# sashajenner/honours

Hardware: AMD Instinct MI355X
Metric: raw-signal MB/s (compress+decompress) (higher is better)
Workload: dtype u16

## Files before the change

honours_amd/csrc/press_huffman.hip:

```cpp

#include "press_internal.h"
#include "press_packed.h"
#include "press_wave.h"
#include <cstddef>
#include <type_traits>

namespace ph {

#ifdef HUF_STAMPS
__device__ unsigned long long g_hstamp[32];
#define HSTAMP_DECL                                             \
	unsigned long long hs_t = __builtin_amdgcn_s_memtime(); \
	unsigned long long hs_acc[8] = { 0, 0, 0, 0, 0, 0, 0, 0 }
#define HSTAMP(i)                                                              \
	do {     \
		__builtin_amdgcn_sched_barrier(0);                             \
		const unsigned long long hs_n = __builtin_amdgcn_s_memtime(); \
		hs_acc[(i) & 7] += hs_n - hs_t;                                \
		hs_t = hs_n;                                                   \
		__builtin_amdgcn_sched_barrier(0);                             \
	} while (0)
#define HSTAMP_FLUSH(base)                                                     \
	do {                                                                   \
		if ((threadIdx.x & 63) == 0)                                   \
			for (int hs_i = 0; hs_i < 8; hs_i++)                   \
				atomicAdd(&g_hstamp[(base) + hs_i], hs_acc[hs_i]); \
	} while (0)
#else
#define HSTAMP_DECL
#define HSTAMP(i)
#define HSTAMP_FLUSH(base)
#endif

constexpr uint32_t HEND = 0xFFFFFFFFu;
constexpr uint32_t R_END = 31;
constexpr int HT = HUF_HT;

__device__ __forceinline__ uint32_t uniform(uint32_t v) { return (uint32_t) __builtin_amdgcn_readfirstlane((int) v); }
__device__ __forceinline__ bool any64(bool c) { return __builtin_amdgcn_ballot_w64(c) != 0; }

__device__ __noinline__ uint32_t trie_code(const HuffDev *hd, uint32_t wnd)
{
	int node = 0;
	uint32_t l = 0;
	while (node >= 0 && hd->leaf[node] < 0 && l < 32) {
		node = hd->child[node][(wnd >> l) & 1u];
		l++;
	}
	if (node < 0 || hd->leaf[node] < 0)
		return 0;
	return (uint32_t) hd->leaf[node] | (l << 8) | (l << 24);
}

template <int RU>
struct HufGeo {
	static constexpr int OWN = 2 * RU;
	static constexpr int NDW = OWN / 32 + 1;
	static constexpr int NCOL = NDW + 1;
};

__device__ __forceinline__ uint32_t clamp_nb(int64_t v)
{
	return v <= 0 ? 0u : (v > 0x7FFFFFFF ? 0x7FFFFFFFu : (uint32_t) v);
}

#ifndef HUF_NO_NT
__device__ __forceinline__ uint4 ld16_pay(const uint8_t *p)
{
	typedef uint32_t u32x4_u __attribute__((ext_vector_type(4), aligned(1)));
	const u32x4_u v = __builtin_nontemporal_load(reinterpret_cast<const u32x4_u *>(p));
	return make_uint4(v.x, v.y, v.z, v.w);
}
__device__ __forceinline__ uint32_t ld4_pay(const uint8_t *p)
{
	typedef uint32_t __attribute__((aligned(1))) u32_u;
	return __builtin_nontemporal_load(reinterpret_cast<const u32_u *>(p));
}
#else
__device__ __forceinline__ uint4 ld16_pay(const uint8_t *p)
{
	uint4 v;
	__builtin_memcpy(&v, p, 16);
	return v;
}
__device__ __forceinline__ uint32_t ld4_pay(const uint8_t *p)
{
	uint32_t v;
	__builtin_memcpy(&v, p, 4);
	return v;
}
#endif

template <int NDW, int S = 64>
__device__ __forceinline__ void col_load(uint32_t *col, const uint8_t *src, int32_t rb0, int32_t lo, int32_t nby)
{
	if (rb0 >= lo && rb0 + 4 * NDW <= nby) {
		const uint8_t *q = src + rb0;
		uint4 t[NDW / 4 ? NDW / 4 : 1];
		uint32_t x[NDW % 4 ? NDW % 4 : 1];
#pragma unroll
		for (int j = 0; j < NDW / 4; j++)
			t[j] = ld16_pay(q + 16 * j);
#pragma unroll
		for (int j = 0; j < NDW % 4; j++)
			x[j] = ld4_pay(q + 4 * (NDW / 4 * 4 + j));
#pragma unroll
		for (int j = 0; j < NDW / 4; j++) {
			col[(4 * j + 0) * S] = t[j].x;
			col[(4 * j + 1) * S] = t[j].y;
			col[(4 * j + 2) * S] = t[j].z;
			col[(4 * j + 3) * S] = t[j].w;
		}
#pragma unroll
		for (int j = 0; j < NDW % 4; j++)
			col[(NDW / 4 * 4 + j) * S] = x[j];
	} else if (nby > lo) {
		uint8_t b[4 * NDW];
#pragma unroll
		for (int i = 0; i < 4 * NDW; i++) {
			const int32_t r = rb0 + i;
			b[i] = src[r < lo ? lo : (r >= nby ? nby - 1 : r)];
		}
#pragma unroll
		for (int j = 0; j < NDW; j++) {
			uint32_t x = 0;
#pragma unroll
			for (int i = 0; i < 4; i++) {
				const int32_t r = rb0 + 4 * j + i;
				x |= (r >= lo && r < nby) ? (uint32_t) b[4 * j + i] << (8 * i) : 0u;
			}
			col[j * S] = x;
		}
	} else {
#pragma unroll
		for (int j = 0; j < NDW; j++)
			col[j * S] = 0;
	}
}

template <int NP>
__device__ __forceinline__ void pay_load(uint32_t (&r)[NP], const uint8_t *src, int32_t rb0, int32_t nby)
{
	if (rb0 + 4 * NP <= nby) {
		const uint8_t *q = src + rb0;
		uint4 t[NP / 4 ? NP / 4 : 1];
		uint32_t x[NP % 4 ? NP % 4 : 1];
#pragma unroll
		for (int j = 0; j < NP / 4; j++)
			t[j] = ld16_pay(q + 16 * j);
#pragma unroll
		for (int j = 0; j < NP % 4; j++)
			x[j] = ld4_pay(q + 4 * (NP / 4 * 4 + j));
#pragma unroll
		for (int j = 0; j < NP / 4; j++) {
			r[4 * j + 0] = t[j].x;
			r[4 * j + 1] = t[j].y;
			r[4 * j + 2] = t[j].z;
			r[4 * j + 3] = t[j].w;
		}
#pragma unroll
		for (int j = 0; j < NP % 4; j++)
			r[NP / 4 * 4 + j] = x[j];
	} else if (nby >= 4) {
		uint32_t d[NP];
#pragma unroll
		for (int j = 0; j < NP; j++) {
			const int32_t p = rb0 + 4 * j;
			d[j] = ld4_pay(src + (p < nby - 4 ? p : nby - 4));
		}
#pragma unroll
		for (int j = 0; j < NP; j++) {
			const int32_t over = rb0 + 4 * j - (nby - 4);
			r[j] = over <= 0 ? d[j] : (over < 4 ? d[j] >> (8 * over) : 0u);
		}
	} else {
		uint32_t x = 0;
		if (rb0 == 0)
			for (int32_t i = 0; i < nby; i++)
				x |= (uint32_t) src[i] << (8 * i);
#pragma unroll
		for (int j = 0; j < NP; j++)
			r[j] = j ? 0u : x;
	}
}

__device__ __forceinline__ int32_t unzz8(uint32_t z) { return (int32_t) (z >> 1) ^ -(int32_t) (z & 1u); }

typedef __attribute__((address_space(3))) const uint32_t *lds_cu32p;
typedef __attribute__((address_space(3))) const uint16_t *lds_cu16p;
typedef __attribute__((address_space(3))) const uint8_t *lds_cu8p;
typedef __attribute__((address_space(3))) uint8_t *lds_u8p;

struct LenTabs {
	alignas(16) uint32_t alut[1 << HUF_LUT_BITS];
	alignas(16) uint16_t flut[1 << HUF_LUT_BITS];
	alignas(16) uint16_t l2ld[HUF_L2_ENTRIES];
};

template <bool TRIE, int S = 64>
__device__ __forceinline__ uint32_t len_scan(const uint32_t *col_, const LenTabs *tabs, const HuffDev *hd, uint32_t start,
					     uint32_t lim, uint32_t nb, uint32_t &cnt, uint32_t &dsum)
{
	const lds_cu32p col = (lds_cu32p) col_;
	const lds_cu32p alut = (lds_cu32p) tabs->alut;
	const lds_cu16p flut = (lds_cu16p) tabs->flut;
	const lds_cu16p l2ld = (lds_cu16p) tabs->l2ld;
	bool bad = start == HEND;
	uint32_t L = lim < nb ? lim : nb;
	if (bad)
		L = 0;
	auto long_ld = [&](uint32_t e, uint32_t wnd) -> uint32_t {
		if (TRIE && e == 0xFFFFFFFFu) {
			const uint32_t t = trie_code(hd, wnd);
			return t ? (((t >> 24) & 31u) | (((uint32_t) unzz8(t & 0xFFu) & 0xFFu) << 8)) : 0u;
		}
		const uint32_t v = l2ld[(e & 0xFFFu) + ((wnd >> HUF_LUT_BITS) & ((1u << ((e >> 12) & 15u)) - 1u))];
		return v == 0xFFFFu ? 0u : v;
	};
	constexpr uint32_t PB = 30;
	const lds_cu32p colm = col - S;
	uint32_t A = (bad ? 0u : start) + PB;
	{
		int32_t LmP = (int32_t) L - HUF_LUT_BITS + (int32_t) PB;
		uint32_t jj = (A >> 5) & 15u;
		uint32_t w0 = colm[__umul24(jj, (uint32_t) S)], w1 = colm[__umul24(jj, (uint32_t) S) + S];
		while ((int32_t) (A & 0x1FFu) <= LmP) {
			const uint32_t pp = A & 0x1FFu;
			{
				const uint32_t w2 = colm[__umul24(jj, (uint32_t) S) + 2 * S];
				const uint32_t wnd = __builtin_amdgcn_alignbit(w1, w0, A);
				const uint32_t e = *(lds_cu32p) ((lds_cu8p) alut + (wnd & (((1u << HUF_LUT_BITS) - 1u) << 2)));
				uint32_t inc = e;
				if ((int32_t) e < 0) {
					const uint32_t ld = long_ld(e, wnd >> 2);
					const uint32_t tot = ld & 0xFFu;
					inc = tot | (1u << HUF_A_CNT) | (((uint32_t) (int32_t) (int8_t) (ld >> 8) & 0x7FFFu) << HUF_A_SUM);
					if (tot - 1u >= L + PB - pp) {
						inc = 0;
						LmP = -1;
					}
				}
				A += inc;
				const uint32_t jn = (A >> 5) & 15u;
				if (jn != jj) {
					w0 = w1;
					w1 = w2;
				}
				jj = jn;
			}
		}
	}
	uint32_t p = (A & 0x1FFu) - PB;
	uint32_t c = (A >> HUF_A_CNT) & 0x7Fu;
	int32_t d = (int32_t) (A << 1) >> 17;
	for (;;) {
		const bool act = p < L;
		if (!any64(act))
			break;
		const uint32_t pp = act ? p : 0u;
		const uint32_t j = pp >> 5;
		const int r0 = (int) __umul24(j, (uint32_t) S);
		const uint32_t wnd = __builtin_amdgcn_alignbit(col[r0 + S], col[r0], pp);
		const uint32_t e = alut[wnd & ((1u << HUF_LUT_BITS) - 1u)];
		const uint32_t f = flut[wnd & ((1u << HUF_LUT_BITS) - 1u)];
		uint32_t tot = e & 15u, n = (e >> HUF_A_CNT) & 15u, len1 = f & 0xFFu;
		int32_t dall = (int32_t) (e << 1) >> 17, d1 = (int32_t) (int8_t) (f >> 8);
		bool fail = false;
		if (any64(act && (int32_t) e < 0)) {
			if (act && (int32_t) e < 0) {
				const uint32_t ld = long_ld(e, wnd);
				tot = len1 = ld & 0xFFu;
				dall = d1 = (int32_t) (int8_t) (ld >> 8);
				fail = tot == 0;
				n = 1;
			}
		}
		const bool fits = pp + tot <= L;
		const bool cut = !fits && pp + len1 > nb;
		if (act && !fail && !cut) {
			p += fits ? tot : len1;
			c += fits ? n : 1u;
			d += fits ? dall : d1;
		}
		if (act && (fail || cut)) {
			bad = true;
			L = 0;
		}
	}
	cnt = c;
	dsum = (uint32_t) d & 0xFFFFu;
	return bad ? HEND : (p >= nb && p < lim ? HEND : p);
}



#ifndef HUF_SYNC_PER_CU
#define HUF_SYNC_PER_CU 2
#endif
#ifndef HUF_RUNUP_EIGHTHS
#define HUF_RUNUP_EIGHTHS 4
#endif
constexpr int WGS = 1024;
constexpr int SYNC_S = 64;

__device__ __forceinline__ uint32_t pack_rec(uint32_t f, uint32_t c, uint32_t d)
{
	return (f == HEND ? R_END : f) | ((c & 0xFFu) << 8) | ((d & 0xFFFFu) << 16);
}

constexpr uint32_t LIST_NONE = 0xFFFFFFFFu;
constexpr uint32_t SYNC_UC = 16;

__device__ __forceinline__ void list_push(uint32_t *list, uint32_t *cnt, uint32_t cap, bool yes, uint32_t value, uint32_t lane)
{
	const unsigned long long m = __ballot(yes);
	if (!m)
		return;
	uint32_t base = 0;
	if (lane == (uint32_t) __builtin_ctzll(m))
		base = atomicAdd(cnt, (uint32_t) __popcll(m));
	base = (uint32_t) __shfl((int) base, __builtin_ctzll(m), 64);
	const uint32_t idx = base + (uint32_t) __popcll(m & ((1ull << lane) - 1ull));
	if (yes && idx < cap)
		list[idx] = value;
}

__device__ __forceinline__ void load_len_tables(const HuffDev *hd, LenTabs *t, uint32_t nthr)
{
	const uint4 *s4 = reinterpret_cast<const uint4 *>(hd->alut);
	uint4 *d4 = reinterpret_cast<uint4 *>(t->alut);
	for (uint32_t i = threadIdx.x; i < (1u << HUF_LUT_BITS) / 4; i += nthr)
		d4[i] = s4[i];
	const uint4 *f4 = reinterpret_cast<const uint4 *>(hd->flut);
	uint4 *g4 = reinterpret_cast<uint4 *>(t->flut);
	for (uint32_t i = threadIdx.x; i < (1u << HUF_LUT_BITS) / 8; i += nthr)
		g4[i] = f4[i];
	const uint4 *t4 = reinterpret_cast<const uint4 *>(hd->l2ld);
	uint4 *u4 = reinterpret_cast<uint4 *>(t->l2ld);
	for (uint32_t i = threadIdx.x; i < (uint32_t) HUF_L2_ENTRIES / 8; i += nthr)
		u4[i] = t4[i];
}


template <int NDW, int S>
__device__ __forceinline__ void col_put(uint32_t *col, const uint32_t *r)
{
	wave_lds_sync();
#pragma unroll
	for (int j = 0; j < NDW; j++)
		col[j * S] = r[j];
	wave_lds_sync();
}

__device__ __forceinline__ unsigned long long spread32(uint32_t x)
{
	unsigned long long v = x;
	v = (v | v << 16) & 0x0000FFFF0000FFFFull;
	v = (v | v << 8) & 0x00FF00FF00FF00FFull;
	v = (v | v << 4) & 0x0F0F0F0F0F0F0F0Full;
	v = (v | v << 2) & 0x3333333333333333ull;
	v = (v | v << 1) & 0x5555555555555555ull;
	return v;
}

template <int RU, bool TRIE>
__global__ __launch_bounds__(WGS, 2 * HUF_SYNC_PER_CU * 2) void k_huf_sync(DecodeArgs a)
{
	constexpr int OWN = HufGeo<RU>::OWN, NDW = HufGeo<RU>::NDW;
	constexpr int W = OWN / 32, NP = 2 * W + 1;
	constexpr int RUNUP = OWN * HUF_RUNUP_EIGHTHS / 8;
	constexpr int S = SYNC_S;
	constexpr uint32_t UP = HT / 128;
	struct Lds {
		LenTabs tabs;
		uint32_t imgs[WGS / 64][(NDW + 2) * S];
	};
	__shared__ __attribute__((aligned(16))) Lds lds;
	__shared__ unsigned long long s_chunk[64];
	__shared__ uint32_t s_ticket;
	auto &imgs = lds.imgs;

	const uint32_t n = min(uniform(a.ctl->nchunks), a.max_htiles);
	const uint32_t nunits = n * UP;
	const uint32_t lane = threadIdx.x & 63;
	if (threadIdx.x == 0)
		s_ticket = 0;
	if (threadIdx.x < 64)
		s_chunk[threadIdx.x] = ~0ull;
	load_len_tables(a.huff, &lds.tabs, WGS);
	__syncthreads();
	uint32_t *img = imgs[threadIdx.x >> 6];
	for (uint32_t i = lane; i < 2 * S; i += 64)
		img[NDW * S + i] = 0;
	uint32_t *col = img + lane;
	HSTAMP_DECL;
	for (;;) {
		uint32_t u = 0;
		if (lane == 0) {
			const uint32_t t = atomicAdd(&s_ticket, 1u);
			const uint32_t c = t / SYNC_UC, slot = t % SYNC_UC;
			unsigned long long *cs = &s_chunk[c & 63u];
			if (slot == 0) {
				u = atomicAdd(&a.ctl->sunits, SYNC_UC);
				__hip_atomic_store(cs, ((unsigned long long) c << 32) | u, __ATOMIC_RELAXED, __HIP_MEMORY_SCOPE_WORKGROUP);
			} else {
				unsigned long long v;
				do {
					v = __hip_atomic_load(cs, __ATOMIC_RELAXED, __HIP_MEMORY_SCOPE_WORKGROUP);
				} while ((uint32_t) (v >> 32) != c);
				u = (uint32_t) v + slot;
			}
		}
		u = uniform(u);
		if (u >= nunits)
			break;
		HSTAMP(0);
		const uint32_t k = u / UP;
		const uint32_t tid = (u % UP) * 128 + 2 * lane;
		const HufTile *dp = a.htiles + k;
		const uint32_t nbits_t = uniform(dp->nbits);
		const uint32_t t = uniform(dp->t_last) & 0x7FFFFFFFu;
		const uint8_t *src = a.in + dp->src;
		const int32_t nby = (int32_t) ((nbits_t + 7) >> 3);
// ... 236 lines not shown
	if (tid == 0) {
		s_cum = 0;
		s_stop = 0xFFFFFFFFu;
		s_refuse = 0;
	}
	__syncthreads();
	{
		uint64_t c = 0;
		for (uint32_t u = tid; u < nu; u += HT)
			c += hw[u].x;
		if (c)
			atomicAdd(&s_cum, (unsigned long long) c);
	}
	const uint32_t want = uniform(a.htiles[k0].want);
	const uint32_t nex = uniform(a.meta[r].nex);
	const uint64_t o0 = a.htiles[k0].low;
	uint32_t *val = a.ex_val + o0;
	const uint32_t *pos = a.ex_pos + o0;
	uint32_t xcum = 0;
	for (uint32_t b = 0; b < nex; b += HT) {
		const uint32_t e = b + tid;
		const uint32_t z = e < nex ? (val[e] & 0xFFFFu) : 0u;
		const uint32_t dl = e < nex ? unzz16(z) : 0u;
		const uint32_t inc = wave_incl_scan_dpp(dl);
		if ((tid & 63) == 63)
			s_w[tid >> 6] = inc;
		__syncthreads();
		uint32_t before = 0, total = 0;
#pragma unroll
		for (int w2 = 0; w2 < HT / 64; w2++) {
			const uint32_t x = s_w[w2];
			if (w2 < (int) (tid >> 6))
				before += x;
			total += x;
		}
		if (e < nex)
			val[e] = z | (((xcum + before + inc - dl) & 0xFFFFu) << 16);
		xcum += total;
		__syncthreads();
	}
	__syncthreads();
	const uint64_t cumall = s_cum;
	const uint32_t nlow = cumall < want ? (uint32_t) cumall : want;
	if (cumall < want) {
		constexpr uint32_t OWN = HufGeo<RU>::OWN;
		const uint64_t nbits0 = a.htiles[k0].nbits;
		const uint64_t nsub64 = (nbits0 + OWN - 1) / OWN;
		const uint32_t nsub = nsub64 < (uint64_t) nt * HT ? (uint32_t) nsub64 : nt * HT;
		const uint8_t *he = a.hend + (uint64_t) k0 * HT;
		for (uint32_t i = tid; i < nsub; i += HT)
			if (he[i] == R_END) {
				atomicMin(&s_stop, i);
				break;
			}
		__syncthreads();
		if (tid == 0 && s_stop != 0xFFFFFFFFu) {
			const uint32_t f = a.hrec[(uint64_t) k0 * HT + s_stop] & 0xFFu;
			if (f != R_END) {
				const HuffDev *hd = a.huff;
				const uint8_t *pay = a.in + a.htiles[k0].src;
				uint64_t p = (uint64_t) s_stop * OWN + f;
				int node = 0;
				for (uint32_t i = 0; i < OWN + 64 && p < nbits0; i++, p++) {
					node = hd->child[node][(pay[p >> 3] >> (p & 7)) & 1u];
					if (node < 0) {
						s_refuse = 1;
						break;
					}
					if (hd->leaf[node] >= 0)
						node = 0;
				}
			}
		}
		__syncthreads();
	}
	const bool refused = s_refuse != 0;
	const bool fused = !refused && nlow >= 1 && (nex == 0 || pos[nex - 1] < nlow + nex);
	const uint32_t zd0 = uniform(a.meta[r].zd0) & 0xFFFFu, q = uniform(a.meta[r].q);
	const uint64_t src0 = a.htiles[k0].src;
	const int64_t nby0 = (int64_t) ((a.htiles[k0].nbits + 7u) >> 3);
	uint64_t cum = 0;
	uint32_t dcum = 0;
	for (uint32_t b = 0; b < nu; b += HT) {
		const uint32_t u = b + tid;
		uint32_t c = 0, dt = 0;
		if (u < nu) {
			const uint2 w = hw[u];
			c = w.x;
			dt = w.y & 0xFFFFu;
		}
		const uint32_t inc = wave_incl_scan_dpp(c);
		const uint32_t dinc = wave_incl_scan_dpp(dt);
		if ((tid & 63) == 63) {
			s_w[tid >> 6] = inc;
			s_wd[tid >> 6] = dinc;
		}
		__syncthreads();
		uint32_t before = 0, total = 0, dbefore = 0, dtotal = 0;
#pragma unroll
		for (int w2 = 0; w2 < HT / 64; w2++) {
			const uint32_t x = s_w[w2], y = s_wd[w2];
			if (w2 < (int) (tid >> 6)) {
				before += x;
				dbefore += y;
			}
			total += x;
			dtotal += y;
		}
		if (u < nu) {
			const uint64_t ob = cum + before + inc - c;
			const uint32_t L0 = ob > 0xFFFFFFFFull ? 0xFFFFFFFFu : (uint32_t) ob;
			const uint32_t quota = L0 >= want ? 0u : (c < want - L0 ? c : want - L0);
			const uint32_t L1 = L0 + quota;
			uint32_t Ea = 0, Eb = 0;
			if (fused && quota) {
				keys_below2(pos, nex, L0, L1, Ea, Eb);
				if (L1 == nlow)
					Eb = nex;
			}
			uint32_t bz = zd0;
			if (L0) {
				bz = unzz16(zd0) + ((dcum + dbefore + dinc - dt) & 0xFFFFu);
				if (Ea) {
					const uint32_t pv = val[Ea - 1];
					bz += (pv >> 16) + unzz16(pv & 0xFFFFu);
				}
				bz &= 0xFFFFu;
			}
			const uint64_t src = src0 + (uint64_t) u * UB;
			const int64_t nby = nby0 - (int64_t) u * UB;
			const uint32_t nbyc = nby <= 0 ? 0u : (nby > (int64_t) HUF_U_NBY ? HUF_U_NBY : (uint32_t) nby);
			uint4 *d = reinterpret_cast<uint4 *>(a.hunit + (uint64_t) k0 * UPT + u);
			d[0] = make_uint4((uint32_t) src, (uint32_t) (src >> 32) | (bz << 16), (uint32_t) o0, (uint32_t) (o0 >> 32));
			d[1] = make_uint4(L0, quota | (nbyc << 14) | ((q & 15u) << 26) | (fused ? 1u << 30 : 0u), Ea, Eb - Ea);
		}
		cum += total;
		dcum += dtotal;
		__syncthreads();
	}
	static_assert(HUF_U_QUOTA >= 64u * 255u, "a unit's quota");
	if (tid == 0) {
		a.meta[r].nlow = nlow;
		if (refused)
			a.meta[r].status = 1;
		if (fused)
			a.hread[2 * r + 1] = nt | HUF_FUSED;
	}
}


constexpr uint32_t EMIT_STG = 4096;

template <bool TRIE>
__device__ __forceinline__ void emit_codes(const uint32_t *col_, const uint32_t *lut_, const uint16_t *lut2_,
					   const HuffDev *hd, uint32_t p, uint32_t nmine, uint8_t *wp_)
{
	const lds_cu32p col = (lds_cu32p) col_;
	const lds_cu8p lut = (lds_cu8p) lut_;
	const lds_cu16p lut2 = (lds_cu16p) lut2_;
	auto long_entry = [&](uint32_t e, uint32_t wnd) -> uint32_t {
		if (TRIE && e == 0xFFFFFFFFu) {
			const uint32_t t = trie_code(hd, wnd);
			return t ? ((t & 0xFFFFFF00u) | ((uint32_t) unzz8(t & 0xFFu) & 0xFFu)) : 0u;
		}
		const uint32_t e2 = lut2[(e & 0xFFFu) + ((wnd >> HUF_LUT_BITS) & ((1u << ((e >> 12) & 15u)) - 1u))];
		return e2 == 0xFFFFu ? 0u : (((uint32_t) unzz8(e2 & 0xFFu) & 0xFFu) | (e2 & 0x1F00u) | ((e2 & 0x1F00u) << 16));
	};
	typedef lds_u8p WP;
	WP w = (WP) wp_;
	const WP wend = w + nmine;
	WP wlim = nmine ? wend - 1 : w;
	constexpr uint32_t PB = 30;
	const lds_cu32p colm = col - 64;
	uint32_t pp = p + PB;
	uint32_t jj = pp >> 5;
	uint32_t w0 = colm[__umul24(jj, 64u)], w1 = colm[__umul24(jj, 64u) + 64];
	while (w < wlim) {
		{
			const uint32_t w2 = colm[__umul24(jj, 64u) + 128];
			const uint32_t wnd = __builtin_amdgcn_alignbit(w1, w0, pp);
			uint32_t e = *(lds_cu32p) (lut + (wnd & (((1u << HUF_LUT_BITS) - 1u) << 2)));
			if (e >= HUF_LONG)
				e = long_entry(e, wnd >> 2);
			w[0] = (uint8_t) e;
			w[1] = (uint8_t) (e >> 16);
			w += 1u + ((e >> 29) & 1u);
			pp += (e >> 8) & 0x1Fu;
			const uint32_t jn = pp >> 5;
			if (jn != jj) {
				w0 = w1;
				w1 = w2;
			}
			jj = jn;
		}
	}
	if (w < wend) {
		const uint32_t wnd = __builtin_amdgcn_alignbit(w1, w0, pp);
		uint32_t e = *(lds_cu32p) (lut + (wnd & (((1u << HUF_LUT_BITS) - 1u) << 2)));
		if (e >= HUF_LONG)
			e = long_entry(e, wnd >> 2);
		w[0] = (uint8_t) e;
	}
}


__device__ __forceinline__ uint32_t lower_bound_u32(const uint32_t *p, uint32_t n, uint32_t key)
{
	uint32_t lo = 0, hi = n;
	while (lo < hi) {
		const uint32_t mid = (lo + hi) >> 1;
		if (p[mid] < key)
			lo = mid + 1;
		else
			hi = mid;
	}
	return lo;
}

template <typename LOWAT, typename BELOW, typename POSAT, typename VALAT>
__device__ __forceinline__ void gather8(LOWAT lowat, BELOW below, POSAT posat, VALAT valat, uint32_t zd0, uint32_t i0,
					uint32_t Ia, uint32_t Ib, uint32_t e_first, uint32_t e_cnt, uint32_t v[4])
{
	v[0] = v[1] = v[2] = v[3] = 0;
	const uint32_t lo = i0 > Ia ? i0 : Ia;
	const uint32_t hi = i0 + 8 < Ib ? i0 + 8 : Ib;
	if (lo >= hi)
		return;
	const uint32_t uf = lo ? lo - 1 : 0;
	uint32_t k = below(uf);
	uint32_t l = uf - e_first - k;
	uint32_t nextpos = k < e_cnt ? posat(k) : 0xFFFFFFFFu;
#pragma unroll
	for (int h = 0; h < 8; h++) {
		const uint32_t i = i0 + h;
		if (i >= lo && i < hi) {
			uint32_t dl;
			if (i == 0) {
				dl = unzz16(zd0);
			} else if (i - 1 == nextpos) {
				dl = unzz16(valat(k) & 0xFFFFu);
				k++;
				nextpos = k < e_cnt ? posat(k) : 0xFFFFFFFFu;
			} else {
				dl = lowat(l) & 0xFFFFu;
				l++;
			}
			v[h >> 1] |= dl << (16 * (h & 1));
		}
	}
}

struct EmitRead {
	const uint32_t *pos, *val;
	int16_t *out;
	uint32_t zd0, q;
};

constexpr uint32_t EMIT_ALIGN = 8;

__device__ __forceinline__ void expand8s(uint2 dd, uint32_t v[4])
{
	typedef short i16x2 __attribute__((ext_vector_type(2)));
	const i16x2 eight = { 8, 8 };
	const uint32_t t[4] = { __builtin_amdgcn_perm(0, dd.x, 0x010c000c), __builtin_amdgcn_perm(0, dd.x, 0x030c020c),
				__builtin_amdgcn_perm(0, dd.y, 0x010c000c), __builtin_amdgcn_perm(0, dd.y, 0x030c020c) };
#pragma unroll
	for (int h = 0; h < 4; h++)
		v[h] = __builtin_bit_cast(uint32_t, __builtin_bit_cast(i16x2, t[h]) >> eight);
}

struct EmitPlan {
	uint32_t L0, L1;
	uint32_t Ea, ecnt;
	uint32_t Ia, Ib;
	uint32_t base;
	uint32_t pe;
};

template <bool BIG>
__device__ __forceinline__ void emit_samples16(const uint8_t *src, uint32_t *exl_, const EmitRead &R, const EmitPlan &P,
					       uint32_t lane)
{
	typedef __attribute__((address_space(3))) uint32_t *lds_u32p;
	const uint32_t L0 = P.L0, L1 = P.L1, Ea = P.Ea, ecnt = P.ecnt, Ia = P.Ia, Ib = P.Ib, pe = P.pe;
	uint32_t base = P.base;
	const lds_u32p exl = (lds_u32p) exl_;
	if (!BIG) {
		uint32_t ve = 0;
		if (ecnt != 0 && lane < ecnt)
			ve = R.val[Ea + lane];
		exl[lane] = pe;
		exl[64 + lane] = ve;
		wave_lds_sync();
	}
	auto ex_below = [&](uint32_t key) -> uint32_t {
		if (BIG)
			return uniform(lower_bound_u32(R.pos + Ea, ecnt, key));
		return (uint32_t) __popcll(__ballot(pe < key));
	};
	auto below = [&](uint32_t key) -> uint32_t {
		if (BIG)
			return lower_bound_u32(R.pos + Ea, ecnt, key);
		uint32_t k = 0;
#pragma unroll
		for (uint32_t st = 32; st; st >>= 1)
			k += exl[k + st - 1] < key ? st : 0u;
		return k + (exl[k] < key ? 1u : 0u);
	};
	auto posat = [&](uint32_t k) -> uint32_t { return BIG ? R.pos[Ea + k] : exl[k]; };
	auto valat = [&](uint32_t k) -> uint32_t { return BIG ? R.val[Ea + k] : exl[64 + k]; };
	const bool shift = uniform(R.q) != 0;
	const u16x2 qq = { (unsigned short) R.q, (unsigned short) R.q };
	const uint32_t *s32 = reinterpret_cast<const uint32_t *>(src);
	for (uint32_t g = Ia & ~(EMIT_ALIGN - 1); g < Ib; g += 1024) {
		const uint32_t i0 = g + lane * 16;
		const uint32_t e0 = ex_below(g ? g - 1 : 0u), e1 = ex_below(g + 1023);
		const bool plain = e0 == e1 && g != 0;
		const bool ragged = g < Ia || g + 1024 > Ib;
		uint32_t v[8];
		if (plain) {
			const bool any = i0 + 16 > Ia && i0 < Ib;
			const int32_t o = any ? (int32_t) (i0 - 1 - Ea - e0 - L0) : 0;
			const int32_t j = o >> 2;
			const uint32_t sh = (uint32_t) (o & 3) * 8u;
			const uint32_t d0 = s32[j], d1 = s32[j + 1], d2 = s32[j + 2], d3 = s32[j + 3], d4 = s32[j + 4];
			uint2 da = make_uint2(__builtin_amdgcn_alignbit(d1, d0, sh), __builtin_amdgcn_alignbit(d2, d1, sh));
			uint2 db = make_uint2(__builtin_amdgcn_alignbit(d3, d2, sh), __builtin_amdgcn_alignbit(d4, d3, sh));
			if (g < Ia) {
				auto mask8 = [&](uint2 &dd, uint32_t ia) {
					const uint32_t lo = Ia > ia ? (Ia - ia < 8 ? Ia - ia : 8u) : 0u;
					const uint64_t m = lo >= 8 ? 0ull : ~((1ull << (8 * lo)) - 1ull);
					dd.x &= (uint32_t) m;
					dd.y &= (uint32_t) (m >> 32);
				};
				mask8(da, i0);
				mask8(db, i0 + 8);
			}
			expand8s(da, v);
			expand8s(db, v + 4);
		} else {
			auto lowat = [&](uint32_t l) -> uint32_t { return (l >= L0 && l < L1) ? (uint32_t) (int32_t) (int8_t) src[l - L0] : 0u; };
			gather8(lowat, below, posat, valat, R.zd0, i0, Ia, Ib, Ea, ecnt, v);
			gather8(lowat, below, posat, valat, R.zd0, i0 + 8, Ia, Ib, Ea, ecnt, v + 4);
		}
		const uint32_t ta = lane_prefix8(v) & 0xFFFFu;
		const uint32_t tb = lane_prefix8(v + 4) & 0xFFFFu;
		const uint32_t tot = (ta + tb) & 0xFFFFu;
		const uint32_t inc = wave_incl_scan_dpp(tot);
		const uint32_t ba = (base + inc - tot) & 0xFFFFu, bb = (ba + ta) & 0xFFFFu;
		const uint32_t ba2 = ba | (ba << 16), bb2 = bb | (bb << 16);
#pragma unroll
		for (int h = 0; h < 4; h++) {
			v[h] = pk_add16(v[h], ba2);
			v[4 + h] = pk_add16(v[4 + h], bb2);
		}
		if (shift) {
#pragma unroll
			for (int h = 0; h < 8; h++)
				v[h] = __builtin_bit_cast(uint32_t, __builtin_bit_cast(u16x2, v[h]) << qq);
		}
#if defined(EMIT_ABL) && EMIT_ABL == 1
		if (R.q == 0x7FFFFFFFu)
#endif
#pragma unroll
		for (int hh = 0; hh < 2; hh++) {
			const uint32_t ia = i0 + 8 * hh;
			if (!ragged || (ia >= Ia && ia + 8 <= Ib)) {
				typedef uint32_t u32x4 __attribute__((ext_vector_type(4)));
				const u32x4 vv = { v[4 * hh], v[4 * hh + 1], v[4 * hh + 2], v[4 * hh + 3] };
#ifdef EMIT_NT_STORES
				__builtin_nontemporal_store(vv, reinterpret_cast<u32x4 *>(R.out + ia));
#else
				*reinterpret_cast<u32x4 *>(R.out + ia) = vv;
#endif
			} else if (ia < Ib && ia + 8 > Ia) {
#pragma unroll
				for (uint32_t h = 0; h < 8; h++)
					if (ia + h >= Ia && ia + h < Ib)
						R.out[ia + h] = (int16_t) (v[4 * hh + (h >> 1)] >> (16 * (h & 1)));
			}
		}
		base += (uint32_t) __builtin_amdgcn_readlane((int) inc, 63);
	}
}

__device__ __forceinline__ uint32_t zz_bytes(uint32_t d)
{
	return ((d << 1) & 0xFEFEFEFEu) ^ (((d >> 7) & 0x01010101u) * 0xFFu);
}

#ifndef EMIT_WG
#define EMIT_WG 512
#endif
#ifndef EMIT_PER_CU
#define EMIT_PER_CU 2
#endif
constexpr int WGE = EMIT_WG;
constexpr uint32_t EMIT_UC = 16;

struct EmitStg {
	uint8_t pre[16];
	uint8_t s[WGE / 64][EMIT_STG];
	uint8_t post[32];
};

template <int RU, bool TRIE>
__global__ __launch_bounds__(WGE) void k_huf_emit(DecodeArgs a)
{
	constexpr int OWN = HufGeo<RU>::OWN, NDW = HufGeo<RU>::NDW, NCOL = HufGeo<RU>::NDW;
	constexpr uint32_t EW = WGE / 64;
	struct Lds {
		alignas(16) uint32_t lut[1 << HUF_LUT_BITS];
		alignas(16) uint16_t lut2[HUF_L2_ENTRIES];
		uint32_t img[EW][NCOL * 64];
		uint32_t pad_row[2 * 64];
		alignas(16) EmitStg stg_all;
		uint32_t exl[EW][128];
	};
	__shared__ __attribute__((aligned(16))) Lds lds;
	auto &lut = lds.lut;
	auto &lut2 = lds.lut2;
	auto &img = lds.img;
	auto &pad_row = lds.pad_row;
	auto &stg_all = lds.stg_all;
	__shared__ unsigned long long s_chunk[64];
	__shared__ uint32_t s_ticket;

	const uint32_t lane = threadIdx.x & 63;
	const uint32_t wv = threadIdx.x >> 6;
	const uint32_t ntiles = min(uniform(a.ctl->nchunks), a.max_htiles);
	const uint32_t nunits = ntiles * (HT / 64);
	if (threadIdx.x == 0) {
		pad_row[0] = 0;
		s_ticket = 0;
	}
	if (threadIdx.x < 64)
		s_chunk[threadIdx.x] = ~0ull;
	{
		const uint4 *s4 = reinterpret_cast<const uint4 *>(a.huff->lut32);
		uint4 *d4 = reinterpret_cast<uint4 *>(lut);
		for (uint32_t i = threadIdx.x; i < (1u << HUF_LUT_BITS) / 4; i += WGE)
			d4[i] = s4[i];
		const uint4 *t4 = reinterpret_cast<const uint4 *>(a.huff->lut2);
		uint4 *u4 = reinterpret_cast<uint4 *>(lut2);
		for (uint32_t i = threadIdx.x; i < (uint32_t) HUF_L2_ENTRIES / 8; i += WGE)
			u4[i] = t4[i];
	}
	uint32_t *col = img[wv] + lane;
	uint8_t *stg = stg_all.s[wv];
	uint32_t *exl = lds.exl[wv];
	__syncthreads();
	auto draw = [&]() -> uint32_t {
		uint32_t u = 0;
		if (lane == 0) {
			const uint32_t t = atomicAdd(&s_ticket, 1u);
			const uint32_t c = t / EMIT_UC, slot = t % EMIT_UC;
			unsigned long long *cs = &s_chunk[c & 63u];
			if (slot == 0) {
				u = atomicAdd(&a.ctl->units, EMIT_UC);
				__hip_atomic_store(cs, ((unsigned long long) c << 32) | u, __ATOMIC_RELAXED, __HIP_MEMORY_SCOPE_WORKGROUP);
			} else {
				unsigned long long v;
				do {
					v = __hip_atomic_load(cs, __ATOMIC_RELAXED, __HIP_MEMORY_SCOPE_WORKGROUP);
				} while ((uint32_t) (v >> 32) != c);
				u = (uint32_t) v + slot;
			}
		}
		return uniform(u);
	};
	static_assert(offsetof(HufUnit, obase) == 16 && offsetof(HufUnit, ecnt) == 28, "the plan is read as eight dwords");
	static_assert(63 * (OWN / 8) + 4 * NDW <= HUF_U_NBY, "HufUnit::qnf's byte count tells whether every lane's bytes lie inside");
	auto fetch_unit = [&](uint32_t u) -> uint32_t {
		uint32_t v = 0;
		if (u < nunits && lane < 8)
			v = reinterpret_cast<const uint32_t *>(a.hunit + u)[lane];
		return v;
	};
	struct Unit {
		uint32_t u, obase, quota, nby, fused, q, bz, ea, ecnt;
		uint64_t srco, roff;
	};
	auto resolve = [&](uint32_t u, uint32_t tv) -> Unit {
		auto at = [&](int i) -> uint32_t { return (uint32_t) __builtin_amdgcn_readlane((int) tv, i); };
		Unit U;
		U.u = u;
		const uint32_t hb = at(1), qnf = at(5);
		U.srco = ((uint64_t) (hb & 0xFFFFu) << 32) | at(0);
		U.bz = hb >> 16;
		U.roff = ((uint64_t) at(3) << 32) | at(2);
		U.obase = at(4);
		U.quota = qnf & HUF_U_QUOTA;
		U.nby = (qnf >> 14) & HUF_U_NBY;
		U.q = (qnf >> 26) & 15u;
		U.fused = qnf >> 30;
		U.ea = at(6);
		U.ecnt = at(7);
		return U;
	};
	struct Stage2 {
		uint32_t pay[NDW];
		uint32_t rec, pe;
		bool fast;
	};
	auto issue2 = [&](const Unit &U, Stage2 &S) {
		const int32_t rb0 = (int32_t) lane * (OWN / 8);
		S.fast = U.nby >= 63 * (OWN / 8) + 4 * NDW;
		const uint8_t *q = a.in + U.srco + rb0;
		if (S.fast) {
			uint4 t[NDW / 4 ? NDW / 4 : 1];
#pragma unroll
			for (int j = 0; j < NDW / 4; j++)
				t[j] = ld16_pay(q + 16 * j);
#pragma unroll
			for (int j = 0; j < NDW % 4; j++)
				S.pay[NDW / 4 * 4 + j] = ld4_pay(q + 4 * (NDW / 4 * 4 + j));
#pragma unroll
			for (int j = 0; j < NDW / 4; j++) {
				S.pay[4 * j + 0] = t[j].x;
				S.pay[4 * j + 1] = t[j].y;
				S.pay[4 * j + 2] = t[j].z;
				S.pay[4 * j + 3] = t[j].w;
			}
		}
		S.rec = a.hrec[(uint64_t) U.u * 64 + lane];
		S.pe = (U.ecnt <= 64 && lane < U.ecnt) ? a.ex_pos[U.roff + U.ea + lane] : 0xFFFFFFFFu;
	};
	auto land2 = [&](const Unit &U, const Stage2 &S) {
		wave_lds_sync();
		if (S.fast) {
#pragma unroll
			for (int j = 0; j < NDW; j++)
				col[j * 64] = S.pay[j];
		} else {
			col_load<NDW>(col, a.in + U.srco, (int32_t) lane * (OWN / 8), 0, (int32_t) U.nby);
		}
		wave_lds_sync();
	};
	HSTAMP_DECL;
	const uint32_t u_first = draw();
	if (u_first >= nunits)
		return;
	Unit U = resolve(u_first, fetch_unit(u_first)), Un = {}, Unn = {};
	Stage2 S, Sn = {};
	issue2(U, S);
	land2(U, S);
	uint32_t u_nxt = draw();
	if (u_nxt < nunits)
		Un = resolve(u_nxt, fetch_unit(u_nxt));
	for (;;) {
		const uint32_t u_nn = draw();
		const uint32_t tv_nn = fetch_unit(u_nn);
		const bool more = u_nxt < nunits;
		if (more)
			issue2(Un, Sn);
		HSTAMP(0);
		const uint32_t rec = S.rec;
		const uint32_t quota = U.quota;
		const uint32_t obase = U.obase;
		const uint64_t roff = U.roff;
		const uint32_t cnt = (rec >> 8) & 0xFFu;
		const uint32_t inc = wave_incl_scan_dpp(cnt);
		const bool fused = U.fused != 0;
		const uint32_t ex = inc - cnt;
		const uint32_t f = rec & 0xFFu;
		const uint32_t p0 = f == R_END ? 0u : f;
		uint32_t nmine = (ex >= quota || f == R_END) ? 0u : (cnt < quota - ex ? cnt : quota - ex);
		nmine = ex >= EMIT_STG ? 0u : (nmine < EMIT_STG - ex ? nmine : EMIT_STG - ex);
		HSTAMP(2);
		{
#if defined(EMIT_ABL) && EMIT_ABL == 3
			if (a.nreads == 0x7FFFFFFFu)
#endif
			emit_codes<TRIE>(col, lut, lut2, a.huff, p0, nmine, stg + ex);
			HSTAMP(3);
			const uint32_t pe = S.pe;
			if (more)
				land2(Un, Sn);
			else
				wave_lds_sync();
			Unn = resolve(u_nn, tv_nn);
			HSTAMP(1);
			if (fused) {
				if (quota) {
					EmitRead R;
					R.pos = a.ex_pos + roff;
					R.val = a.ex_val + roff;
					R.out = a.sig + roff;
					R.zd0 = U.bz;
					R.q = U.q;
					EmitPlan P;
					P.L0 = obase;
					P.L1 = obase + quota;
					P.Ea = U.ea;
					P.ecnt = U.ecnt;
					P.Ia = obase ? obase + U.ea + 1 : 0u;
					P.Ib = P.L1 + U.ea + U.ecnt + 1;
					P.base = obase ? U.bz : 0u;
					P.pe = pe;
					HSTAMP(4);
#if defined(EMIT_ABL) && EMIT_ABL == 2
					if (a.nreads == 0x7FFFFFFFu)
#endif
					{
						if (U.ecnt <= 64)
							emit_samples16<false>(stg, exl, R, P, lane);
						else {
							emit_samples16<true>(stg, exl, R, P, lane);
							__builtin_amdgcn_s_waitcnt(0x0F70);
						}
					}
					HSTAMP(5);
				}
			} else {
				uint8_t *dst = a.low + roff + obase;
				for (uint32_t o = lane * 16; o < quota; o += 64 * 16) {
					uint4 v = *reinterpret_cast<const uint4 *>(stg + o);
					v = make_uint4(zz_bytes(v.x), zz_bytes(v.y), zz_bytes(v.z), zz_bytes(v.w));
					if (o + 16 <= quota) {
						__builtin_memcpy(dst + o, &v, 16);
					} else {
						const uint32_t vv[4] = { v.x, v.y, v.z, v.w };
						for (uint32_t b = 0; o + b < quota; b++)
							dst[o + b] = (uint8_t) (vv[b >> 2] >> (8 * (b & 3)));
					}
				}
			}
			wave_lds_sync();
		}
		HSTAMP(6);
		if (!more)
			break;
		U = Un;
		S = Sn;
		Un = Unn;
		u_nxt = u_nn;
	}
	HSTAMP_FLUSH(8);
}


constexpr uint32_t TILES_RPW = 16;
__global__ __launch_bounds__(64) void k_huff_tiles(DecodeArgs a)
{
	const uint32_t lane = threadIdx.x;
	const uint32_t r = lane < TILES_RPW ? blockIdx.x * TILES_RPW + lane : 0xFFFFFFFFu;
	const uint32_t minlen = a.huff->minlen, maxlen = a.huff->maxlen;
	const uint32_t OWN = minlen >= 4 ? 256u : minlen >= 2 ? 128u : 64u;
	const uint64_t TB = (uint64_t) HT * OWN;
	uint32_t nt = 0;
	if (r < a.nreads && a.meta[r].status == 0) {
		const ReadMeta *m = a.meta + r;
		const uint32_t hdr = m->hdr + m->seclen + 4;
		const uint64_t nbytes64 = a.in_len[r] - hdr;
		const uint64_t nbits = 8ull * (nbytes64 > 0x1FFFFFFFull ? 0x1FFFFFFFull : nbytes64);
		const uint64_t need = (uint64_t) m->nlow * maxlen;
		const uint64_t span = nbits < need ? nbits : need;
		nt = (uint32_t) ((span + TB - 1) / TB);
	}
	uint32_t inc = nt;
#pragma unroll
	for (int dd = 1; dd < 64; dd <<= 1) {
		const uint32_t t2 = (uint32_t) __shfl_up((int) inc, dd, 64);
		if ((int) lane >= dd)
			inc += t2;
	}
	const uint32_t wsum = (uint32_t) __shfl((int) inc, 63, 64);
	uint32_t base = 0;
	if (lane == 0 && wsum)
		base = atomicAdd(&a.ctl->nchunks, wsum);
	base = (uint32_t) __shfl((int) base, 0, 64) + inc - nt;
	if (r < a.nreads) {
		if (base + nt > a.max_htiles)
			nt = base < a.max_htiles ? a.max_htiles - base : 0;
		a.hread[2 * r] = base;
		a.hread[2 * r + 1] = nt;
		a.hmin[r] = 0xFFFFFFFFu;
	}
	uint64_t src0 = 0, low0 = 0, nbits = 0;
	uint32_t want = 0;
	if (nt) {
		const ReadMeta *m = a.meta + r;
		const uint32_t hdr = m->hdr + m->seclen + 4;
		const uint64_t nbytes64 = a.in_len[r] - hdr;
		nbits = 8ull * (nbytes64 > 0x1FFFFFFFull ? 0x1FFFFFFFull : nbytes64);
		src0 = a.in_off[r] + hdr;
		low0 = a.off[r];
		want = m->nlow;
	}
	unsigned long long todo = __ballot(nt != 0);
	while (todo) {
		const int rr = __builtin_ctzll(todo);
		todo &= todo - 1;
		const uint32_t r_nt = (uint32_t) __shfl((int) nt, rr, 64), r_base = (uint32_t) __shfl((int) base, rr, 64);
		const uint32_t r_read = (uint32_t) __shfl((int) r, rr, 64), r_want = (uint32_t) __shfl((int) want, rr, 64);
		const uint64_t r_src = ((uint64_t) (uint32_t) __shfl((int) (src0 >> 32), rr, 64) << 32) | (uint32_t) __shfl((int) src0, rr, 64);
		const uint64_t r_low = ((uint64_t) (uint32_t) __shfl((int) (low0 >> 32), rr, 64) << 32) | (uint32_t) __shfl((int) low0, rr, 64);
		const uint64_t r_bits = ((uint64_t) (uint32_t) __shfl((int) (nbits >> 32), rr, 64) << 32) | (uint32_t) __shfl((int) nbits, rr, 64);
		for (uint32_t t = lane; t < r_nt; t += 64) {
			HufTile d;
			d.src = r_src + t * (TB / 8);
			d.low = r_low;
			d.nbits = (uint32_t) (r_bits - t * TB);
			d.t_last = t | (t + 1 == r_nt ? 0x80000000u : 0u);
			d.read = r_read;
			d.want = r_want;
			a.htiles[r_base + t] = d;
		}
	}
}

#ifndef HUF_FIX_ROUNDS
#define HUF_FIX_ROUNDS 4
#endif
#ifdef HUF_STAMPS
}
extern "C" int press_hip_huf_stamps(unsigned long long *dst, uint32_t nwords)
{
	unsigned long long z[32] = { 0 };
	if (hipDeviceSynchronize() != hipSuccess ||
	    hipMemcpyFromSymbol(dst, HIP_SYMBOL(ph::g_hstamp), (nwords < 32 ? nwords : 32) * 8) != hipSuccess ||
	    hipMemcpyToSymbol(HIP_SYMBOL(ph::g_hstamp), z, sizeof z) != hipSuccess)
		return -1;
	return 0;
}
namespace ph {
#endif
// ... 46 lines not shown
```

honours_amd/csrc/press_table.hip:

```cpp

#include <stdlib.h>

#include <vector>

#include "press_host.h"

using namespace ph;

static inline int32_t unzz8(uint32_t z) { return (int32_t) (z >> 1) ^ -(int32_t) (z & 1u); }

int ph::upload_table(const uint32_t len[256], const uint64_t bits[256])
{
	if (g.have_table && !memcmp(len, g.tlen, sizeof g.tlen) && !memcmp(bits, g.tbits, sizeof g.tbits))
		return 0;
	std::vector<HuffDev> hv(1);
	HuffDev &h = hv[0];
	memset(&h, 0xFF, sizeof h);
	int nnodes = 1, ncoded = 0;
	bool needs_trie = false;
	for (int s = 0; s < 256; s++) {
		const uint32_t l = len[s];
		if (l > 24)
			return set_error(PRESS_HIP_EARG, "Huffman table: symbol %d has a code of %u bits (at most 24)", s, l);
		if (l == 0) {
			h.enc[s] = 0;
			continue;
		}
		ncoded++;
		h.enc[s] = (uint32_t) (bits[s] & 0xFFFFFFu) | (l << 24);
		int p = 0;
		for (uint32_t k = 0; k < l; k++) {
			const int b = (int) ((bits[s] >> k) & 1);
			if (h.leaf[p] >= 0)
				return set_error(PRESS_HIP_EARG, "Huffman table: not a prefix code");
			if (h.child[p][b] < 0) {
				if (nnodes >= 1024)
					return set_error(PRESS_HIP_EARG, "Huffman table: too many nodes");
				h.child[p][b] = (int16_t) nnodes++;
			}
			p = h.child[p][b];
		}
		if (h.child[p][0] >= 0 || h.child[p][1] >= 0)
			return set_error(PRESS_HIP_EARG, "Huffman table: not a prefix code");
		h.leaf[p] = (int16_t) s;
		if (l <= (uint32_t) HUF_LUT_BITS) {
			const uint32_t step = 1u << l;
			for (uint32_t i = (uint32_t) bits[s] & (step - 1); i < (1u << HUF_LUT_BITS); i += step)
				h.lut[i] = (uint16_t) (s | (l << 8));
		}
	}
	{
		int nid = 0;
		uint32_t used = 0;
		int id_of[1 << HUF_LUT_BITS];
		for (int i = 0; i < (1 << HUF_LUT_BITS); i++)
			id_of[i] = -1;
		uint32_t depth[256] = { 0 };
		int prefix_of[256];
		for (int s = 0; s < 256; s++) {
			if (len[s] <= (uint32_t) HUF_LUT_BITS)
				continue;
			const int pfx = (int) (bits[s] & ((1u << HUF_LUT_BITS) - 1));
			if (id_of[pfx] < 0 && nid < HUF_L2_IDS) {
				prefix_of[nid] = pfx;
				id_of[pfx] = nid++;
			}
			if (id_of[pfx] >= 0 && len[s] - HUF_LUT_BITS > depth[id_of[pfx]])
				depth[id_of[pfx]] = len[s] - HUF_LUT_BITS;
		}
		for (uint32_t d = 32; d >= 1; d--) {
			for (int id = 0; id < nid; id++) {
				if (depth[id] != d)
					continue;
				if (d > 12 || used + (1u << d) > (uint32_t) HUF_L2_ENTRIES)
					continue;
				h.l2off[id] = (uint16_t) used;
				h.l2bits[id] = (uint8_t) d;
				h.lut[prefix_of[id]] = (uint16_t) (0x8000u | (uint32_t) id);
				used += 1u << d;
			}
		}
		for (int s = 0; s < 256; s++) {
			if (len[s] <= (uint32_t) HUF_LUT_BITS)
				continue;
			const int pfx = (int) (bits[s] & ((1u << HUF_LUT_BITS) - 1));
			const int id = id_of[pfx];
			if (id < 0 || h.lut[pfx] != (uint16_t) (0x8000u | (uint32_t) id))
				continue;
			const uint32_t rest = (uint32_t) (bits[s] >> HUF_LUT_BITS), rl = len[s] - HUF_LUT_BITS;
			for (uint32_t i = rest; i < (1u << depth[id]); i += 1u << rl)
				h.lut2[h.l2off[id] + i] = (uint16_t) (s | (len[s] << 8));
		}
		needs_trie = used > HUF_L2_NONE;
		for (int s = 0; s < 256; s++) {
			if (len[s] <= (uint32_t) HUF_LUT_BITS)
				continue;
			const int pfx = (int) (bits[s] & ((1u << HUF_LUT_BITS) - 1));
			const int id = id_of[pfx];
			if (id < 0 || h.lut[pfx] != (uint16_t) (0x8000u | (uint32_t) id))
				needs_trie = true;
		}
		for (int i = 0; i < HUF_L2_ENTRIES; i++) {
			const uint32_t e2 = h.lut2[i];
			h.l2ld[i] = e2 == 0xFFFFu ? (uint16_t) 0xFFFFu : (uint16_t) ((e2 >> 8) | ((unzz8(e2 & 0xFFu) & 0xFFu) << 8));
		}
	}
	for (uint32_t i = 0; i < (1u << HUF_LUT_BITS); i++) {
		const uint16_t e1 = h.lut[i];
		if (e1 == 0xFFFFu) {
			h.lut32[i] = needs_trie ? 0xFFFFFFFFu : (HUF_LONG | HUF_L2_NONE);
		} else if (e1 & 0x8000u) {
			const uint32_t id = e1 & 0xFFu;
			h.lut32[i] = HUF_LONG | ((uint32_t) h.l2bits[id] << 12) | h.l2off[id];
		} else {
			const uint32_t s1 = (uint32_t) unzz8(e1 & 0xFFu) & 0xFFu, l1 = e1 >> 8;
			uint32_t v = s1 | (l1 << 8) | (l1 << 24);
			const uint32_t rest = (uint32_t) HUF_LUT_BITS - l1;
			const uint16_t e2 = h.lut[i >> l1];
			if (e2 != 0xFFFFu && !(e2 & 0x8000u) && (uint32_t) (e2 >> 8) <= rest)
				v = s1 | ((l1 + (e2 >> 8)) << 8) | (((uint32_t) unzz8(e2 & 0xFFu) & 0xFFu) << 16) | (l1 << 24) | HUF_TWO;
			h.lut32[i] = v;
		}
	}
	for (uint32_t i = 0; i < (1u << HUF_LUT_BITS); i++) {
		uint32_t pos = 0, n = 0, len1 = 0;
		int32_t d1 = 0, dsum = 0;
		for (;;) {
			const uint16_t e1 = h.lut[i >> pos];
			if (e1 == 0xFFFFu || (e1 & 0x8000u) || pos + (uint32_t) (e1 >> 8) > (uint32_t) HUF_LUT_BITS)
				break;
			const int32_t d = (int32_t) unzz8(e1 & 0xFFu);
			if (!n) {
				len1 = e1 >> 8;
				d1 = d;
			}
			dsum += d;
			pos += e1 >> 8;
			n++;
			if (pos == (uint32_t) HUF_LUT_BITS || n == HUF_M_MAXN)
				break;
		}
		const uint16_t e0 = h.lut[i];
		if (n)
			h.mlut[i] = pos | (n << 4) | (len1 << 8) | (((uint32_t) d1 & 0xFFu) << 12) | (((uint32_t) dsum & 0x7FFu) << 20);
		else if (e0 != 0xFFFFu && (e0 & 0x8000u))
			h.mlut[i] = HUF_MLONG | (uint32_t) h.l2off[e0 & 0xFFu] | ((uint32_t) h.l2bits[e0 & 0xFFu] << 12);
		else
			h.mlut[i] = needs_trie ? 0xFFFFFFFFu : (HUF_MLONG | HUF_L2_NONE);
		h.alut[i] = n ? (pos | (n << HUF_A_CNT) | (((uint32_t) dsum & 0x7FFFu) << HUF_A_SUM)) : h.mlut[i];
		h.flut[i] = n ? (uint16_t) (len1 | (((uint32_t) d1 & 0xFFu) << 8)) : (uint16_t) 0;
	}
	if (!ncoded)
		return set_error(PRESS_HIP_EARG, "Huffman table: no symbol has a code");
	h.minlen = 64;
	h.maxlen = 0;
	for (int s = 0; s < 256; s++) {
		if (!len[s])
			continue;
		h.minlen = len[s] < h.minlen ? len[s] : h.minlen;
		h.maxlen = len[s] > h.maxlen ? len[s] : h.maxlen;
	}
	HIPCHK(hipStreamSynchronize(g.stream()));
	if (g.huff.reserve(sizeof(HuffDev)))
		return PRESS_HIP_EHIP;
	HIPCHK(hipMemcpy(g.huff.p, &h, sizeof h, hipMemcpyHostToDevice));
	memcpy(g.tlen, len, sizeof g.tlen);
	memcpy(g.tbits, bits, sizeof g.tbits);
	g.tmin = h.minlen;
	g.tmax = h.maxlen;
	g.table_trie = needs_trie;
	g.have_table = true;
	return 0;
}

namespace {
int parse_table_file(FILE *fp, uint32_t len[256], uint64_t bits[256]);
}

extern "C" int press_hip_set_table(const uint32_t len[256], const uint64_t bits[256])
{
	API_ENTER;
	return upload_table(len, bits);
}

extern "C" int press_hip_load_table_file(const char *path)
{
	uint32_t len[256];
	uint64_t bits[256];
	FILE *fp = fopen(path, "rb");
	if (!fp)
		return set_error(PRESS_HIP_EARG, "cannot open %s", path);
	int rc = parse_table_file(fp, len, bits);
	fclose(fp);
	if (rc)
		return rc;
	return press_hip_set_table(len, bits);
}


namespace {

huffman_node *new_node(bool leaf, unsigned char sym)
{
	huffman_node *p = (huffman_node *) calloc(1, sizeof *p);
	if (!p)
		return nullptr;
	p->isLeaf = leaf ? 1 : 0;
	if (leaf)
		p->symbol = sym;
	return p;
}

int parse_table_file(FILE *fp, uint32_t len[256], uint64_t bits[256])
{
	unsigned char hd[8];
	memset(len, 0, 256 * sizeof len[0]);
	memset(bits, 0, 256 * sizeof bits[0]);
	if (fread(hd, 1, 8, fp) != 8)
		return set_error(PRESS_HIP_EARG, "Huffman table: short header");
	uint32_t count = ((uint32_t) hd[0] << 24) | ((uint32_t) hd[1] << 16) | ((uint32_t) hd[2] << 8) | hd[3];
	if (count > 256)
		return set_error(PRESS_HIP_EARG, "Huffman table: %u entries", count);
	for (uint32_t i = 0; i < count; i++) {
		int sym = fgetc(fp), nb = fgetc(fp);
		if (sym == EOF || nb == EOF || nb == 0 || nb > 64)
			return set_error(PRESS_HIP_EARG, "Huffman table: bad entry %u", i);
		unsigned char code[8] = { 0 };
		if (fread(code, 1, (size_t) (nb + 7) / 8, fp) != (size_t) (nb + 7) / 8)
			return set_error(PRESS_HIP_EARG, "Huffman table: truncated");
		uint64_t b = 0;
		for (int k = 0; k < nb; k++)
			if (code[k / 8] & (1u << (k % 8)))
				b |= 1ull << k;
		len[sym] = (uint32_t) nb;
		bits[sym] = b;
	}
	return 0;
}

void collect_codes(const huffman_node *p, uint64_t code, uint32_t depth, uint32_t len[256], uint64_t bits[256])
{
	if (!p || depth > 64)
		return;
	if (p->isLeaf) {
		len[p->symbol] = depth;
		bits[p->symbol] = code;
		return;
	}
	collect_codes(p->zero, code, depth + 1, len, bits);
	collect_codes(p->one, code | (depth < 64 ? 1ull << depth : 0), depth + 1, len, bits);
}

}

int ph::table_from_encoder(SymbolEncoder *se)
{
	API_LOCK;
// ... 126 lines not shown
```

Baseline: 864,400.

## Add flut-only fast scan path and unify second-level Huffman table lookups

```diff
diff --git a/honours_amd/csrc/press_huffman.hip b/honours_amd/csrc/press_huffman.hip
--- a/honours_amd/csrc/press_huffman.hip
+++ b/honours_amd/csrc/press_huffman.hip
@@ -26,10 +26,16 @@
 			for (int hs_i = 0; hs_i < 8; hs_i++)                   \
 				atomicAdd(&g_hstamp[(base) + hs_i], hs_acc[hs_i]); \
 	} while (0)
+#define HCOUNT(i)                                                                       \
+	do {                                                                            \
+		if ((threadIdx.x & 63) == (uint32_t) __builtin_ctzll(__ballot(true)))   \
+			atomicAdd(&g_hstamp[i], 1ull);                                  \
+	} while (0)
 #else
 #define HSTAMP_DECL
 #define HSTAMP(i)
 #define HSTAMP_FLUSH(base)
+#define HCOUNT(i)
 #endif
 
 constexpr uint32_t HEND = 0xFFFFFFFFu;
@@ -190,6 +196,12 @@
 typedef __attribute__((address_space(3))) const uint16_t *lds_cu16p;
 typedef __attribute__((address_space(3))) const uint8_t *lds_cu8p;
 typedef __attribute__((address_space(3))) uint8_t *lds_u8p;
+
+__device__ __forceinline__ uint32_t l2_entry(lds_cu16p l2ld, uint32_t e, uint32_t wnd, uint32_t sh)
+{
+	const uint32_t x = __builtin_amdgcn_ubfe(wnd, sh + HUF_LUT_BITS, (e >> 12) & 15u);
+	return *(lds_cu16p) ((lds_cu8p) l2ld + (((e & 0xFFFu) + x) << 1));
+}
 
 struct LenTabs {
 	alignas(16) uint32_t alut[1 << HUF_LUT_BITS];
@@ -209,15 +221,16 @@
 	uint32_t L = lim < nb ? lim : nb;
 	if (bad)
 		L = 0;
-	auto long_ld = [&](uint32_t e, uint32_t wnd) -> uint32_t {
+	auto long_ld = [&](uint32_t e, uint32_t wnd, uint32_t sh) -> uint32_t {
 		if (TRIE && e == 0xFFFFFFFFu) {
-			const uint32_t t = trie_code(hd, wnd);
+			const uint32_t t = trie_code(hd, wnd >> sh);
 			return t ? (((t >> 24) & 31u) | (((uint32_t) unzz8(t & 0xFFu) & 0xFFu) << 8)) : 0u;
 		}
-		const uint32_t v = l2ld[(e & 0xFFFu) + ((wnd >> HUF_LUT_BITS) & ((1u << ((e >> 12) & 15u)) - 1u))];
-		return v == 0xFFFFu ? 0u : v;
+		return l2_entry(l2ld, e, wnd, sh);
 	};
 	constexpr uint32_t PB = 30;
+	constexpr uint32_t LD_INC = 0x08010C00u;
+	static_assert(HUF_A_SUM == 16, "LD_INC places the delta at bit 16");
 	const lds_cu32p colm = col - S;
 	uint32_t A = (bad ? 0u : start) + PB;
 	{
@@ -232,9 +245,9 @@
 				const uint32_t e = *(lds_cu32p) ((lds_cu8p) alut + (wnd & (((1u << HUF_LUT_BITS) - 1u) << 2)));
 				uint32_t inc = e;
 				if ((int32_t) e < 0) {
-					const uint32_t ld = long_ld(e, wnd >> 2);
+					const uint32_t ld = long_ld(e, wnd, 2);
 					const uint32_t tot = ld & 0xFFu;
-					inc = tot | (1u << HUF_A_CNT) | (((uint32_t) (int32_t) (int8_t) (ld >> 8) & 0x7FFFu) << HUF_A_SUM);
+					inc = __builtin_amdgcn_perm(0u, ld, LD_INC) | (1u << HUF_A_CNT);
 					if (tot - 1u >= L + PB - pp) {
 						inc = 0;
 						LmP = -1;
@@ -249,6 +262,33 @@
 				jj = jn;
 			}
 		}
+		HCOUNT(24);
+		if (!any64(start < L && nb < lim + 2 * HUF_LUT_BITS)) {
+			HCOUNT(27);
+			uint32_t LT = L + PB;
+			while ((A & 0x1FFu) < LT) {
+				HCOUNT(26);
+				const uint32_t w2 = colm[__umul24(jj, (uint32_t) S) + 2 * S];
+				const uint32_t wnd = __builtin_amdgcn_alignbit(w1, w0, A);
+				const uint32_t f = *(lds_cu16p) ((lds_cu8p) flut + ((wnd >> 1) & (((1u << HUF_LUT_BITS) - 1u) << 1)));
+				uint32_t inc = __builtin_amdgcn_perm(0u, f, LD_INC);
+				if (f == 0) {
+					const uint32_t ld = long_ld(*(lds_cu32p) ((lds_cu8p) alut + (wnd & (((1u << HUF_LUT_BITS) - 1u) << 2))), wnd, 2);
+					inc = __builtin_amdgcn_perm(0u, ld, LD_INC);
+					if ((ld & 0xFFu) == 0) {
+						inc = 0u - (1u << HUF_A_CNT);
+						LT = 0;
+					}
+				}
+				A += inc + (1u << HUF_A_CNT);
+				const uint32_t jn = (A >> 5) & 15u;
+				if (jn != jj) {
+					w0 = w1;
+					w1 = w2;
+				}
+				jj = jn;
+			}
+		}
 	}
 	uint32_t p = (A & 0x1FFu) - PB;
 	uint32_t c = (A >> HUF_A_CNT) & 0x7Fu;
@@ -257,6 +297,7 @@
 		const bool act = p < L;
 		if (!any64(act))
 			break;
+		HCOUNT(25);
 		const uint32_t pp = act ? p : 0u;
 		const uint32_t j = pp >> 5;
 		const int r0 = (int) __umul24(j, (uint32_t) S);
@@ -268,7 +309,7 @@
 		bool fail = false;
 		if (any64(act && (int32_t) e < 0)) {
 			if (act && (int32_t) e < 0) {
-				const uint32_t ld = long_ld(e, wnd);
+				const uint32_t ld = long_ld(e, wnd, 0);
 				tot = len1 = ld & 0xFFu;
 				dall = d1 = (int32_t) (int8_t) (ld >> 8);
 				fail = tot == 0;
@@ -811,19 +852,18 @@
 constexpr uint32_t EMIT_STG = 4096;
 
 template <bool TRIE>
-__device__ __forceinline__ void emit_codes(const uint32_t *col_, const uint32_t *lut_, const uint16_t *lut2_,
+__device__ __forceinline__ void emit_codes(const uint32_t *col_, const uint32_t *lut_, const uint16_t *l2ld_,
 					   const HuffDev *hd, uint32_t p, uint32_t nmine, uint8_t *wp_)
 {
 	const lds_cu32p col = (lds_cu32p) col_;
 	const lds_cu8p lut = (lds_cu8p) lut_;
-	const lds_cu16p lut2 = (lds_cu16p) lut2_;
+	const lds_cu16p l2ld = (lds_cu16p) l2ld_;
 	auto long_entry = [&](uint32_t e, uint32_t wnd) -> uint32_t {
 		if (TRIE && e == 0xFFFFFFFFu) {
-			const uint32_t t = trie_code(hd, wnd);
+			const uint32_t t = trie_code(hd, wnd >> 2);
 			return t ? ((t & 0xFFFFFF00u) | ((uint32_t) unzz8(t & 0xFFu) & 0xFFu)) : 0u;
 		}
-		const uint32_t e2 = lut2[(e & 0xFFFu) + ((wnd >> HUF_LUT_BITS) & ((1u << ((e >> 12) & 15u)) - 1u))];
-		return e2 == 0xFFFFu ? 0u : (((uint32_t) unzz8(e2 & 0xFFu) & 0xFFu) | (e2 & 0x1F00u) | ((e2 & 0x1F00u) << 16));
+		return __builtin_amdgcn_perm(0u, l2_entry(l2ld, e, wnd, 2), 0x000C0001u);
 	};
 	typedef lds_u8p WP;
 	WP w = (WP) wp_;
@@ -840,7 +880,7 @@
 			const uint32_t wnd = __builtin_amdgcn_alignbit(w1, w0, pp);
 			uint32_t e = *(lds_cu32p) (lut + (wnd & (((1u << HUF_LUT_BITS) - 1u) << 2)));
 			if (e >= HUF_LONG)
-				e = long_entry(e, wnd >> 2);
+				e = long_entry(e, wnd);
 			w[0] = (uint8_t) e;
 			w[1] = (uint8_t) (e >> 16);
 			w += 1u + ((e >> 29) & 1u);
@@ -857,7 +897,7 @@
 		const uint32_t wnd = __builtin_amdgcn_alignbit(w1, w0, pp);
 		uint32_t e = *(lds_cu32p) (lut + (wnd & (((1u << HUF_LUT_BITS) - 1u) << 2)));
 		if (e >= HUF_LONG)
-			e = long_entry(e, wnd >> 2);
+			e = long_entry(e, wnd);
 		w[0] = (uint8_t) e;
 	}
 }
@@ -1070,7 +1110,7 @@
 	constexpr uint32_t EW = WGE / 64;
 	struct Lds {
 		alignas(16) uint32_t lut[1 << HUF_LUT_BITS];
-		alignas(16) uint16_t lut2[HUF_L2_ENTRIES];
+		alignas(16) uint16_t l2ld[HUF_L2_ENTRIES];
 		uint32_t img[EW][NCOL * 64];
 		uint32_t pad_row[2 * 64];
 		alignas(16) EmitStg stg_all;
@@ -1078,7 +1118,7 @@
 	};
 	__shared__ __attribute__((aligned(16))) Lds lds;
 	auto &lut = lds.lut;
-	auto &lut2 = lds.lut2;
+	auto &l2ld = lds.l2ld;
 	auto &img = lds.img;
 	auto &pad_row = lds.pad_row;
 	auto &stg_all = lds.stg_all;
@@ -1100,8 +1140,8 @@
 		uint4 *d4 = reinterpret_cast<uint4 *>(lut);
 		for (uint32_t i = threadIdx.x; i < (1u << HUF_LUT_BITS) / 4; i += WGE)
 			d4[i] = s4[i];
-		const uint4 *t4 = reinterpret_cast<const uint4 *>(a.huff->lut2);
-		uint4 *u4 = reinterpret_cast<uint4 *>(lut2);
+		const uint4 *t4 = reinterpret_cast<const uint4 *>(a.huff->l2ld);
+		uint4 *u4 = reinterpret_cast<uint4 *>(l2ld);
 		for (uint32_t i = threadIdx.x; i < (uint32_t) HUF_L2_ENTRIES / 8; i += WGE)
 			u4[i] = t4[i];
 	}
@@ -1231,7 +1271,7 @@
 #if defined(EMIT_ABL) && EMIT_ABL == 3
 			if (a.nreads == 0x7FFFFFFFu)
 #endif
-			emit_codes<TRIE>(col, lut, lut2, a.huff, p0, nmine, stg + ex);
+			emit_codes<TRIE>(col, lut, l2ld, a.huff, p0, nmine, stg + ex);
 			HSTAMP(3);
 			const uint32_t pe = S.pe;
 			if (more)
diff --git a/honours_amd/csrc/press_table.hip b/honours_amd/csrc/press_table.hip
--- a/honours_amd/csrc/press_table.hip
+++ b/honours_amd/csrc/press_table.hip
@@ -102,7 +102,7 @@
 		}
 		for (int i = 0; i < HUF_L2_ENTRIES; i++) {
 			const uint32_t e2 = h.lut2[i];
-			h.l2ld[i] = e2 == 0xFFFFu ? (uint16_t) 0xFFFFu : (uint16_t) ((e2 >> 8) | ((unzz8(e2 & 0xFFu) & 0xFFu) << 8));
+			h.l2ld[i] = e2 == 0xFFFFu ? (uint16_t) 0 : (uint16_t) ((e2 >> 8) | ((unzz8(e2 & 0xFFu) & 0xFFu) << 8));
 		}
 	}
 	for (uint32_t i = 0; i < (1u << HUF_LUT_BITS); i++) {
```

Measured after the change: 890,800 (median of 4 runs). 3.1% higher.
